# casys-kaist/CoVA

Hardware: AMD Instinct MI355X
Metric: compressed-domain frames/sec (BlobNet+bboxcc) at 1080p b=256 (higher is better)
Workload: dtype f16

## Files before the change

cova_amd/_lib.py:

```python
from __future__ import annotations

import ctypes as C
import os

import numpy as np

_HERE = os.path.dirname(os.path.abspath(__file__))
LIB_PATH = os.path.join(_HERE, "libcovahip.so")

OK = 0
MEM_HOST, MEM_DEVICE = 0, 1
AU_DELTA_UNIT, AU_DISCONT, AU_DROPPABLE = 1, 2, 4


class CovahipError(RuntimeError):
    def __init__(self, status: int, where: str, detail: str = ""):
        self.status = status
        try:
            text = lib().covahip_strerror(status).decode()
        except AttributeError:
            text = "error"
        msg = f"{where}: {text} (status {status})"
        if detail:
            msg += f" [{detail}]"
# ... 208 lines not shown
    "covahip_train_create": (C.c_int, [_P, C.POINTER(TrainCfg), _P, _SZ, C.POINTER(_P)]),
    "covahip_train_step": (C.c_int, [_P, _P, _P, C.c_int, C.c_float, C.POINTER(C.c_float), C.c_int]),
    "covahip_train_metrics": (C.c_int, [_P, C.POINTER(C.c_int64)]),
    "covahip_train_weights": (C.c_int, [_P, _P, _SZ, C.POINTER(_SZ)]),
    "covahip_train_grads": (C.c_int, [_P, _P, _SZ]),
    "covahip_train_create_set": (C.c_int, [_P, C.POINTER(TrainCfg), C.c_int, _P, _P, _P, C.POINTER(_P)]),
    "covahip_train_num_models": (C.c_int, [_P, C.POINTER(C.c_int)]),
    "covahip_train_step_set": (C.c_int, [_P, _P, _P, _P, _P, _P, C.c_int]),
    "covahip_train_metrics_m": (C.c_int, [_P, C.c_int, C.POINTER(C.c_int64)]),
    "covahip_train_weights_m": (C.c_int, [_P, C.c_int, _P, _SZ, C.POINTER(_SZ)]),
    "covahip_train_grads_m": (C.c_int, [_P, C.c_int, _P, _SZ]),
    "covahip_train_eval": (C.c_int, [_P, _P, _P, C.c_int, _P, _P, C.POINTER(TrainEvalResult), C.c_int]),
    "covahip_train_eval_set": (C.c_int, [_P, _P, _P, _P, _P, _P, C.POINTER(TrainEvalResult), C.c_int]),
    "covahip_train_state_size": (C.c_int, [_P, C.POINTER(_SZ)]),
    "covahip_train_save_state": (C.c_int, [_P, C.c_uint64, _P, _SZ, C.POINTER(_SZ)]),
    "covahip_train_load_state": (C.c_int, [_P, _P, _SZ, C.POINTER(C.c_uint64)]),
    "covahip_train_set_plan": (C.c_int, [_P, C.POINTER(TrainPlan)]),
    "covahip_train_get_plan": (C.c_int, [_P, C.POINTER(TrainPlan)]),
    "covahip_train_set_post": (C.c_int, [_P, C.c_int, C.POINTER(BlobNetPost)]),
    "covahip_train_get_post": (C.c_int, [_P, C.c_int, C.POINTER(C.c_float), _P, C.POINTER(C.c_int)]),
    "covahip_train_destroy": (None, [_P]),
    "covahip_train_data_create": (C.c_int, [_P, C.c_int, C.c_int, C.c_int64, C.POINTER(_P)]),
    "covahip_train_data_append": (C.c_int, [_P, _P, _P, C.c_int, C.c_int, C.POINTER(C.c_int64)]),
    "covahip_train_data_frames": (C.c_int, [_P, C.POINTER(C.c_int64)]),
    "covahip_train_data_gather": (C.c_int, [_P, _P, C.c_int, _P, _P, C.c_int]),
    "covahip_train_data_destroy": (None, [_P]),
    "covahip_train_step_data": (C.c_int, [_P, _P, _P, C.c_int, C.c_float, C.POINTER(C.c_float)]),
    "covahip_train_step_set_data": (C.c_int, [_P, _P, _P, _P, _P, _P]),
    "covahip_train_eval_data": (C.c_int, [_P, _P, _P, C.c_int, _P, _P, C.POINTER(TrainEvalResult), C.c_int]),
    "covahip_train_eval_set_data": (C.c_int, [_P, _P, _P, _P, _P, _P, C.POINTER(TrainEvalResult), C.c_int]),
    "covahip_post_sweep": (C.c_int, [_P, C.POINTER(SweepCfg), _P, _P, C.c_int, C.c_int, _P, _P, _P, C.POINTER(SweepResult)]),
    "covahip_post_heat_begin": (C.c_int, [_P, C.POINTER(HeatCfg)]),
    "covahip_post_heat_add": (C.c_int, [_P, _P, _P, C.c_int, C.c_int]),
    "covahip_post_heat_end": (C.c_int, [_P, _P, _P, _P, C.POINTER(C.c_int64)]),
    "covahip_monitor_begin": (C.c_int, [_P, C.POINTER(MonitorCfg)]),
    "covahip_monitor_add": (C.c_int, [_P, _P, _P, _P, _P, C.c_int, C.c_int]),
    "covahip_monitor_read": (C.c_int, [_P, C.c_int, _P, _P, _P, _P, _P, _P, C.POINTER(C.c_int64), C.POINTER(C.c_int64)]),
    "covahip_monitor_end": (C.c_int, [_P]),
    "covahip_mog_default_cfg": (None, [C.POINTER(MogCfg)]),
    "covahip_mog_create": (C.c_int, [_P, C.POINTER(MogCfg), C.POINTER(_P)]),
    "covahip_mog_create_grid": (C.c_int, [_P, C.POINTER(MogCfg), C.c_int, C.POINTER(_P)]),
    "covahip_mog_dims": (C.c_int, [_P, C.POINTER(C.c_int32), C.POINTER(C.c_int32), C.POINTER(C.c_int32), C.POINTER(C.c_int32)]),
    "covahip_mog_apply": (C.c_int, [_P, _P, C.c_int, _P, _P, C.c_int]),
    "covahip_mog_yuv_tight": (C.c_int, [_P, C.c_int, C.c_int, C.POINTER(MogYuv)]),
    "covahip_mog_apply_yuv": (C.c_int, [_P, C.POINTER(MogYuv), _P, C.c_int, _P, _P, C.c_int]),
    "covahip_mog_reset": (C.c_int, [_P, C.c_int]),
    "covahip_mog_destroy": (None, [_P]),
}

DEV_PROTOTYPES = {
    "covahip_blobnet_set_impl": (C.c_int, [_P, C.c_int]),
    "covahip_bboxcc_set_wave_cap": (C.c_int, [_P, C.c_int]),
    "covahip_blobnet_set_enc_plan": (C.c_int, [_P, C.c_int, C.c_int, C.c_int]),
    "covahip_dev_clock_mhz": (C.c_int, [_P, C.c_int, C.POINTER(C.c_float)]),
    "covahip_dev_graph_probe": (C.c_int, [_P, _P, C.c_int, _P, C.c_int, C.c_int, _P, _P, C.c_int, _P, C.c_int, C.POINTER(C.c_float),
                                          C.POINTER(C.c_float)]),
    "covahip_dev_bboxcc_overflow": (C.c_int, [_P, C.POINTER(C.c_int32)]),
    "covahip_dev_blobnet_tail_form": (C.c_int, [_P, C.POINTER(C.c_int)]),
    "covahip_dev_pipe_queue_plan": (C.c_int, [_P, C.POINTER(C.c_int), C.POINTER(C.c_int)]),
    "covahip_dev_blobnet_buffer": (C.c_int, [_P, C.c_int, C.c_int, C.POINTER(C.c_void_p), C.POINTER(C.c_size_t), C.POINTER(C.c_int32)]),
    "covahip_dev_mog_masks": (C.c_int, [_P, _P, _P, _SZ, C.POINTER(C.c_int)]),
    "covahip_dev_mog_state": (C.c_int, [_P, C.c_int, _P, _P, _P, _P, C.POINTER(C.c_int64)]),
    "covahip_dev_mog_set_stage_budget": (C.c_int, [_P, _SZ]),
    "covahip_dev_mog_post_masks": (C.c_int, [_P, _P, C.c_int, _P]),
    "covahip_dev_mog_set_post_form": (C.c_int, [_P, C.c_int, C.c_int]),
    "covahip_dev_mog_band_plan": (C.c_int, [C.c_int, C.c_int, C.POINTER(C.c_int), C.POINTER(C.c_int), C.POINTER(C.c_size_t)]),
    "covahip_dev_monitor_slice": (C.c_int, [_P, C.c_int]),
    "covahip_dev_heat_set_stage": (C.c_int, [_P, _SZ]),
    "covahip_dev_train_data_set_stage": (C.c_int, [_P, _SZ]),
}

_lib = None


def lib() -> C.CDLL:
    global _lib
    if _lib is None:
        san = os.environ.get("COVAHIP_HOST_SAN_LIB")
        if san:
            L = C.CDLL(san)
            for name, (res, args) in list(PROTOTYPES.items()) + list(DEV_PROTOTYPES.items()):
                fn = getattr(L, name, None)
                if fn is not None:
                    fn.restype = res
                    fn.argtypes = args
            _lib = L
            return _lib
        if not os.path.exists(LIB_PATH):
            raise ImportError(
                f"{LIB_PATH} not found: build it with `python -c 'import __graft_entry__ as g; g.build()'` "
                "or `make -C cova_amd/csrc` -- cova_amd has no CPU fallback")
        L = C.CDLL(LIB_PATH)
        for name, (res, args) in list(PROTOTYPES.items()) + list(DEV_PROTOTYPES.items()):
            fn = getattr(L, name)
            fn.restype = res
            fn.argtypes = args
        _lib = L
    return _lib


def check(status: int, where: str, ctx=None) -> None:
    if status != OK:
        detail = ""
        if ctx is not None and status == 3:
            detail = lib().covahip_last_hip_error(ctx).decode()
        raise CovahipError(status, where, detail)
# ... 1 lines not shown
```

cova_amd/csrc/blobnet.hip:

```cpp
#include <algorithm>
#include <cmath>
#include <cstdlib>
#include <cstring>
#include <vector>

#include "blobnet.h"
#include "covahip_dev.h"

static void free_model(covahip_ctx *ctx, covahip_blobnet *m) {
    if (!m) return;
    blobnet_release_mfma(ctx, m);
    if (m->d_post) hipFree(m->d_post);
    for (BnWorkspace &ws : m->ws) {
        for (int i = 0; i <= BN_LEVELS; i++)
            if (ws.act[i]) hipFree(ws.act[i]);
        for (int j = 0; j < BN_LEVELS; j++)
            if (ws.dact[j]) hipFree(ws.dact[j]);
        if (ws.pbuf) hipFree(ws.pbuf);
        if (ws.part) hipFree(ws.part);
        ws.index.release();
        ws.models.release();
        ws.areas.release();
    }
    delete m;
// ... 325 lines not shown
    m->post_thr[model] = post ? post->logit_thresh : 0.f;
    m->post_keep[model].clear();
    if (post && post->keep) {
        m->post_keep[model].resize(hw);
        for (size_t i = 0; i < hw; i++) m->post_keep[model][i] = post->keep[i] ? 1 : 0;
    }
    return commit_post(ctx, m);
}

int covahip_blobnet_set_area(covahip_ctx *ctx, int model, int area_thresh) {
    if (!ctx) return COVAHIP_ERR_INVALID_ARG;
    covahip_blobnet *m = ctx->blobnet;
    if (!m) return COVAHIP_ERR_NOT_LOADED;
    if (model < 0 || model >= m->n_models || area_thresh < 0) return COVAHIP_ERR_INVALID_ARG;
    COVAHIP_CHECK_HIP(ctx, hipSetDevice(ctx->device));
    if (int rc = covahip_sync_all(ctx)) return rc;
    m->post_area[model] = area_thresh;
    return commit_post(ctx, m);
}

int covahip_blobnet_get_area(covahip_ctx *ctx, int model, int *area_thresh) {
    if (!ctx || !area_thresh) return COVAHIP_ERR_INVALID_ARG;
    covahip_blobnet *m = ctx->blobnet;
    if (!m) return COVAHIP_ERR_NOT_LOADED;
    if (model < 0 || model >= m->n_models) return COVAHIP_ERR_INVALID_ARG;
    *area_thresh = m->post_area[model];
    return COVAHIP_OK;
}

int covahip_blobnet_get_post(covahip_ctx *ctx, int model, float *logit_thresh, uint8_t *keep_or_null, int *has_keep) {
    if (!ctx) return COVAHIP_ERR_INVALID_ARG;
    covahip_blobnet *m = ctx->blobnet;
    if (!m) return COVAHIP_ERR_NOT_LOADED;
    if (model < 0 || model >= m->n_models) return COVAHIP_ERR_INVALID_ARG;
    const std::vector<uint8_t> &keep = m->post_keep[model];
    if (logit_thresh) *logit_thresh = m->post_thr[model];
    if (has_keep) *has_keep = keep.empty() ? 0 : 1;
    if (keep_or_null) {
        const size_t hw = (size_t)m->H * m->W;
        if (keep.empty()) std::memset(keep_or_null, 1, hw);
        else std::memcpy(keep_or_null, keep.data(), hw);
    }
    return COVAHIP_OK;
}

int covahip_blobnet_macs_per_frame(covahip_ctx *ctx, int64_t *macs) {
    if (!ctx || !macs) return COVAHIP_ERR_INVALID_ARG;
    if (!ctx->blobnet) return COVAHIP_ERR_NOT_LOADED;
    *macs = ctx->blobnet->macs_per_frame;
    return COVAHIP_OK;
}

int covahip_blobnet_set_enc_plan(covahip_ctx *ctx, int level, int nbands, int nbuf) {
    if (!ctx || level < 1 || level > 3 || nbands < 0 || nbands > 64 || (nbands && nbuf != 1 && nbuf != 2)) return COVAHIP_ERR_INVALID_ARG;
    ctx->enc_plan[level].nbands = nbands;
    ctx->enc_plan[level].nbuf = nbands ? nbuf : 0;
    return COVAHIP_OK;
}

int covahip_blobnet_set_impl(covahip_ctx *ctx, int impl) {
    if (!ctx || !ctx->blobnet) return COVAHIP_ERR_NOT_LOADED;
    if (impl != 1 && (impl < 4 || impl > 10)) return COVAHIP_ERR_INVALID_ARG;
    ctx->blobnet->fuse_dec = impl != 4;
    ctx->blobnet->enc1_tile16 = impl != 5;
    ctx->blobnet->enc_rowtiles = impl != 6;
    ctx->blobnet->fuse_enc23 = impl == 7 ? 0 : impl == 8 ? 2 : 1;
    ctx->blobnet->tail_part = impl != 9;
    ctx->blobnet->tail_rows = impl != 10;
    return COVAHIP_OK;
}

static int filter_placed(covahip_ctx *ctx, covahip_blobnet *m, const uint8_t *d_src, int n_frames, const int32_t *stack_index,
                         int batch, int area_thresh, covahip_box *d_boxes, int32_t *d_counts, int max_boxes, float *d_logits,
                         uint8_t *d_mask, bool packed = false, const uint8_t *model_ids = nullptr) {
    if (!d_mask) {
        CtxLane &l = ctx->lane();
        int rc = covahip_ensure_buffer(ctx, &l.cc_scratch, &l.cc_scratch_bytes, (size_t)batch * m->H * m->W);
        if (rc) return rc;
        d_mask = (uint8_t *)l.cc_scratch;
    }
    BnInput in;
    if (n_frames > 0) {
        int rc = prepare_frames(ctx, m, m->ws[ctx->cur_lane], d_src, n_frames, stack_index, batch, in, model_ids);
        if (rc) return rc;
        in.packed = packed;
    } else {
        in.stack = d_src;
    }
    int rc = filter_dev(ctx, in, batch, d_logits, d_mask, true, area_thresh, d_boxes, d_counts, max_boxes, n_frames > 0 ? nullptr : model_ids);
    if (rc == COVAHIP_OK && batch > 0 && ctx->mon && ctx->mon->attached && !ctx->mon_suspended)
        rc = covahip_monitor_hook(ctx, d_mask, d_counts, d_boxes, max_boxes, model_ids, batch);
    return rc;
}

static int filter_any(covahip_ctx *ctx, const uint8_t *src, int n_frames, const int32_t *stack_index, int batch,
                      int area_thresh, covahip_box *boxes, int32_t *counts, int max_boxes, float *logits, uint8_t *mask,
                      int mem_kind, const uint8_t *model_ids = nullptr) {
    if (!ctx || batch < 0 || max_boxes < 0 || n_frames < 0) return COVAHIP_ERR_INVALID_ARG;
    covahip_blobnet *m = ctx->blobnet;
    if (!m) return COVAHIP_ERR_NOT_LOADED;
    if (batch == 0) return COVAHIP_OK;
    if (!src || !counts || (!boxes && max_boxes > 0) || batch > m->max_batch) return COVAHIP_ERR_INVALID_ARG;
    if (int rc = check_model_ids(m, model_ids, batch)) return rc;
    COVAHIP_CHECK_HIP(ctx, hipSetDevice(ctx->device));
    const bool by_frames = n_frames > 0;
    const size_t hw = (size_t)m->H * m->W;
    const size_t in_bytes = by_frames ? (size_t)n_frames * hw * 4 : (size_t)batch * BN_T * hw * 4;
// ... 223 lines not shown
```

cova_amd/csrc/blobnet_mfma.hip:

```cpp
#include <algorithm>
#include <cmath>
#include <cstdlib>
#include <cstring>
#include <mutex>
#include <type_traits>
#include <utility>
#include <vector>

#include "bboxcc_body.h"
#include "bboxcc_wave.h"
#include "blobnet.h"
#include "covahip_dev.h"

typedef _Float16 half8 __attribute__((ext_vector_type(8)));
typedef _Float16 half4 __attribute__((ext_vector_type(4)));
typedef float f32x16 __attribute__((ext_vector_type(16)));
typedef float f32x4 __attribute__((ext_vector_type(4)));
typedef _Float16 half2v __attribute__((ext_vector_type(2)));

namespace {

constexpr float BN_EPS = 1e-3f;
constexpr int WG = 256;

// ... 239 lines not shown
    }
}

#ifdef PHASE_TIMING
__device__ unsigned long long g_phase[80];
#define PHASE_MARK(i)                                                     \
    do {                                                                  \
        const unsigned long long now_ = __builtin_amdgcn_s_memrealtime(); \
        ph_[i] += now_ - last_;                                           \
        last_ = now_;                                                     \
    } while (0)
#else
#define PHASE_MARK(i) do { } while (0)
#endif
#if defined(PHASE_TIMING) || defined(WGSPAN_ONLY)
__device__ unsigned long long g_wgspan[6][1024][4];
#define WGSPAN_BEGIN() const unsigned long long wg_t0_ = __builtin_amdgcn_s_memrealtime(), wg_c0_ = __builtin_amdgcn_s_memtime()
#define WGSPAN_END(kid)                                                                          \
    do {                                                                                         \
        if (threadIdx.x == 0 && blockIdx.x < 1024) {                                             \
            g_wgspan[kid][blockIdx.x][0] = wg_t0_;                                               \
            g_wgspan[kid][blockIdx.x][1] = __builtin_amdgcn_s_memrealtime();                     \
            g_wgspan[kid][blockIdx.x][2] = __builtin_amdgcn_s_getreg(4 | (0 << 6) | (31 << 11)); \
            g_wgspan[kid][blockIdx.x][3] = __builtin_amdgcn_s_memtime() - wg_c0_;                \
        }                                                                                        \
    } while (0)
#else
#define WGSPAN_BEGIN() do { } while (0)
#define WGSPAN_END(kid) do { } while (0)
#endif
#ifdef WGSPAN_ONLY
__device__ unsigned long long g_itemspan[3][1024][4][4];
#define ITEM_MARK(j) do { if (it_n_ < 4) it_t_[it_n_][j] = __builtin_amdgcn_s_memrealtime(); } while (0)
#else
#define ITEM_MARK(j) do { } while (0)
#endif
constexpr int WG0 = 512;
struct Enc0pArgs {
    const uint8_t *in;
    __half *out;
    const half8 *wfrag;
    const float *epi;
    int F, H, W, Hp, Wp, Ho, Wo, oy, ox;
    int nbands, TC;
    uint32_t mWp, mNb, mW4;
    int scr_off;
    const uint8_t *model_ids;
    uint32_t mstride;
};
template <bool ALLPOS, bool PACKED, bool MS = false>
__global__ __launch_bounds__(WG0, 4) void enc0p_mfma(Enc0pArgs p) {
    extern __shared__ __attribute__((aligned(16))) uint8_t smem[];
    WGSPAN_BEGIN();
    const int tid = threadIdx.x, lane = tid & 63, wave = tid >> 6;
    const int TC = p.TC;
    half8 be0 = p.wfrag[lane], be1 = p.wfrag[64 + lane];
    half8 bo0 = p.wfrag[128 + lane], bo1 = p.wfrag[192 + lane];
    const int co = lane & 15;
    float e0 = p.epi[co], e1 = p.epi[16 + co], e2 = p.epi[32 + co];
    [[maybe_unused]] uint32_t moff_cur = 0;
    const int m = lane & 15, g = lane >> 4;
    const uint32_t lc0 = (uint32_t)((((m & 1) + (g >> 1)) * TC + 2 * (m >> 1) + 2 * (g & 1)) * 8);
    const uint32_t lc1 = (uint32_t)((((m & 1) + 2) * TC + 2 * (m >> 1) + 2 * (g & 1)) * 8);
    const int n_items = p.F * p.nbands;
    for (int item = blockIdx.x; item < n_items; item += gridDim.x) {
        const int f = fdiv(item, p.mNb), band = item - f * p.nbands;
        if constexpr (MS) {
            const uint32_t mo = model_off<MS>(p.model_ids, p.mstride, f);
            if (mo != moff_cur) {
                moff_cur = mo;
                const half8 *wf = at_model(p.wfrag, mo);
                const float *ep = at_model(p.epi, mo);
                be0 = wf[lane]; be1 = wf[64 + lane]; bo0 = wf[128 + lane]; bo1 = wf[192 + lane];
                e0 = ep[co]; e1 = ep[16 + co]; e2 = ep[32 + co];
            }
        }
        const int y0 = 2 * ((band * p.Hp) / p.nbands);
        const int rows = 2 * (((band + 1) * p.Hp) / p.nbands) - y0;
        const int n2 = rows + 2;
        lds_barrier();
        {
            const int W4 = p.W >> 2;
            const int per_t = n2 * W4;
            const uint8_t *fb = p.in + (size_t)f * p.H * p.W * (PACKED ? 2 : 4);
            uint4 v[2];
            int dsto[2];
#pragma unroll
            for (int k = 0; k < 2; k++) {
                const int i = tid + k * WG0;
                dsto[k] = -1;
                v[k] = make_uint4(0, 0, 0, 0);
                if (i < per_t) {
                    const int r = fdiv(i, p.mW4), c4 = i - r * W4;
                    const int y = y0 - 1 + r;
                    dsto[k] = r * TC * 8 + 16 + c4 * 32;
                    if (y >= 0 && y < p.H) {
                        if constexpr (PACKED) {
                            const uint2 w = *reinterpret_cast<const uint2 *>(fb + ((size_t)y * p.W + c4 * 4) * 2);
                            v[k].x = w.x; v[k].y = w.y;
                        } else {
                            v[k] = *reinterpret_cast<const uint4 *>(fb + ((size_t)y * p.W + c4 * 4) * 4);
                        }
                    }
                }
            }
            const half2v clip = {(_Float16)1030.f, (_Float16)1030.f}, off = {(_Float16)1024.f, (_Float16)1024.f};
#pragma unroll
            for (int k = 0; k < 2; k++) {
                if (dsto[k] >= 0) {
                    uint32_t o[8];
                    if constexpr (PACKED) {
                        const uint32_t pw[2] = {v[k].x, v[k].y};
#pragma unroll
                        for (int q = 0; q < 4; q++) {
                            const uint32_t r = (pw[q >> 1] >> (16 * (q & 1))) & 0xFFFFu;
                            const uint32_t c01 = 0x64006400u | (r & 7u) | (((r >> 3) & 7u) << 16);
                            const uint32_t c23 = 0x64006400u | ((r >> 6) & 7u);
                            o[2 * q] = __builtin_bit_cast(uint32_t, __builtin_bit_cast(half2v, c01) - off);
                            o[2 * q + 1] = __builtin_bit_cast(uint32_t, __builtin_bit_cast(half2v, c23) - off);
                        }
                    } else {
                        const uint32_t px[4] = {v[k].x, v[k].y, v[k].z, v[k].w};
#pragma unroll
                        for (int q = 0; q < 4; q++) {
                            const uint32_t c01 = __builtin_amdgcn_perm(0x64646464u, px[q], 0x05010500u);
                            const uint32_t c23 = __builtin_amdgcn_perm(0x64646464u, px[q], 0x05030502u);
                            const half2v h01 = __builtin_elementwise_min(__builtin_bit_cast(half2v, c01), clip) - off;
                            const half2v h23 = __builtin_elementwise_min(__builtin_bit_cast(half2v, c23), clip) - off;
                            o[2 * q] = __builtin_bit_cast(uint32_t, h01);
                            o[2 * q + 1] = __builtin_bit_cast(uint32_t, h23);
                        }
                    }
                    uint8_t *d = smem + dsto[k];
                    *reinterpret_cast<uint4 *>(d) = make_uint4(o[0], o[1], o[2], o[3]);
                    *reinterpret_cast<uint4 *>(d + 16) = make_uint4(o[4], o[5], o[6], o[7]);
                }
            }
            for (int i = tid; i < n2 * 2; i += WG0)
                *reinterpret_cast<uint4 *>(smem + (i >> 1) * TC * 8 + ((i & 1) ? (p.W + 2) * 8 : 0)) = make_uint4(0, 0, 0, 0);
        }
        lds_barrier();
        const int nhalf = (p.Wp + 31) >> 5;
        const int ngroups = (rows / 2) * nhalf;
        uint8_t *const scr = smem + p.scr_off + wave * 1024;
        __half *const ob = p.out + (size_t)f * p.Ho * p.Wo * 16;
        int g_wy = 0, g_h = wave;
        for (int grp = wave; grp < ngroups; grp += WG0 / 64, g_h += WG0 / 64) {
            while (g_h >= nhalf) { g_h -= nhalf; g_wy++; }
            const uint32_t gbase = (uint32_t)(((2 * g_wy) * TC + 64 * g_h) * 8);
            const uint8_t *const a0 = smem + (gbase + lc0), *const a1 = smem + (gbase + lc1);
#pragma unroll
            for (int k = 0; k < 4; k++) {
                const half8 ae0 = *reinterpret_cast<const half8 *>(__builtin_assume_aligned(a0 + k * 128, 16));
                const half8 ae1 = *reinterpret_cast<const half8 *>(__builtin_assume_aligned(a1 + k * 128, 16));
                const half8 ao0 = *reinterpret_cast<const half8 *>(__builtin_assume_aligned(a0 + k * 128 + 16, 16));
                const half8 ao1 = *reinterpret_cast<const half8 *>(__builtin_assume_aligned(a1 + k * 128 + 16, 16));
                f32x4 ce = {0.f, 0.f, 0.f, 0.f}, co_ = {0.f, 0.f, 0.f, 0.f};
                ce = __builtin_amdgcn_mfma_f32_16x16x32_f16(ae0, be0, ce, 0, 0, 0);
                co_ = __builtin_amdgcn_mfma_f32_16x16x32_f16(ao0, bo0, co_, 0, 0, 0);
                ce = __builtin_amdgcn_mfma_f32_16x16x32_f16(ae1, be1, ce, 0, 0, 0);
                co_ = __builtin_amdgcn_mfma_f32_16x16x32_f16(ao1, bo1, co_, 0, 0, 0);
                _Float16 *sw = reinterpret_cast<_Float16 *>(scr + (k * 8 + 2 * g) * 32) + co;
                float v0 = pool4<ALLPOS>(ce[0], ce[1], co_[0], co_[1], e0, e1, e2);
                float v1 = pool4<ALLPOS>(ce[2], ce[3], co_[2], co_[3], e0, e1, e2);
                asm volatile("" : "+v"(v0), "+v"(v1));
                sw[0] = (_Float16)v0;
                sw[16] = (_Float16)v1;
            }
            __builtin_amdgcn_fence(__ATOMIC_RELEASE, "wavefront");
            __builtin_amdgcn_wave_barrier();
            __builtin_amdgcn_fence(__ATOMIC_ACQUIRE, "wavefront");
            const int owx = 32 * g_h + (lane >> 1);
            if (owx < p.Wp) {
                const int gy = y0 / 2 + g_wy + p.oy, gx = owx + p.ox;
                *reinterpret_cast<uint4 *>(ob + (gy * p.Wo + gx) * 16 + 8 * (lane & 1)) =
                    *reinterpret_cast<const uint4 *>(scr + lane * 16);
            }
            __builtin_amdgcn_fence(__ATOMIC_RELEASE, "wavefront");
            __builtin_amdgcn_wave_barrier();
        }
    }
    WGSPAN_END(5);
}

template <int CIN, int COUT, int TPAR, int OCC, int NWV, bool WIDE, bool ALLPOS, bool PRE = false, int TSZ = 0, bool MS = false>
__global__ __launch_bounds__(NWV * 64, OCC) void enc_mfma(EncArgs p) {
    constexpr int WGS = NWV * 64;
    constexpr int NT = COUT / 32, MG = NWV / NT, KC = CIN / 16, KSTEPS = 9 * KC;
    constexpr int CPP = CIN / 8, PS = CIN * 2;
    constexpr int AD = CIN == 32 ? 8 : 0;
    extern __shared__ __attribute__((aligned(16))) uint8_t smem[];
    const int tid = threadIdx.x, lane = tid & 63, wave = tid >> 6;
    const int ntile = wave % NT, mgroup = wave / NT;
    const int TR = p.TR, TC = p.TC;
    const int tsz = TSZ > 0 ? TSZ : TR * TC * PS;
    static_assert(TSZ == 0 || (TSZ % 16 == 0 && (TPAR - 1) * TSZ < 65536 && !PRE), "T-slice offsets must fit a DS instruction's offset field");

    WGSPAN_BEGIN();
#ifdef PHASE_TIMING
    unsigned long long ph_[9] = {0, 0, 0, 0, 0, 0, 0, 0, 0}, last_ = __builtin_amdgcn_s_memrealtime();
    asm volatile("s_waitcnt lgkmcnt(0)" ::: "memory");
#endif
    auto mlp_own = [&](uint8_t *base, int band_, const TmixW &tmp) {
        const int n2_ = 2 * (((band_ + 1) * p.Hp) / p.nbands) - 2 * ((band_ * p.Hp) / p.nbands) + 2;
        const int nchunk = n2_ * TC * CPP;
        for (int sidx = tid; sidx < nchunk; sidx += WGS) {
            half8 v[BN_T], o[BN_T];
#pragma unroll
            for (int t = 0; t < BN_T; t++) v[t] = *reinterpret_cast<const half8 *>(base + t * tsz + sidx * 16);
#pragma unroll
            for (int j0 = 0; j0 < 8; j0 += 4) {
                half4 pb[4];
                f32x4 r[4];
#pragma unroll
                for (int j = 0; j < 4; j++) pb[j] = half4{v[0][j0 + j], v[1][j0 + j], v[2][j0 + j], v[3][j0 + j]};
                tmix4f<4>(tmp, pb, r);
#pragma unroll
                for (int j = 0; j < 4; j++)
#pragma unroll
                    for (int t = 0; t < BN_T; t++) o[t][j0 + j] = (_Float16)r[j][t];
            }
#pragma unroll
            for (int t = 0; t < BN_T; t++) *reinterpret_cast<half8 *>(base + t * tsz + sidx * 16) = o[t];
        }
    };
    auto stage = [&](int sb, int sband, uint8_t *dst, int ll) {
        const int sy0 = 2 * ((sband * p.Hp) / p.nbands);
        const int sn2 = 2 * (((sband + 1) * p.Hp) / p.nbands) - sy0 + 2;
        int fidx[BN_T] = {0, 1, 2, 3};
        if constexpr (PRE) {
            typedef int i32x4 __attribute__((ext_vector_type(4)));
            typedef const __attribute__((address_space(4))) i32x4 *const_i32x4_ptr;
            if (p.pidx) {
// ... 1988 lines not shown

void blobnet_release_mfma(covahip_ctx *, covahip_blobnet *m) {
    if (m->d_prepared) hipFree(m->d_prepared);
    m->d_prepared = nullptr;
    delete m->prep;
    m->prep = nullptr;
}

namespace {

struct Fwd {
    covahip_ctx *ctx;
    const covahip_blobnet *m;
    const Prepared *pr;
    BnWorkspace &ws;
    const BnInput &inp;
    int batch;
    const uint8_t *prep;
    uint32_t mstride;
    bool ms;
    bool dry;
    bool by_frames;
    int num_cu;
    const uint8_t *d_frames;
    int n_frames;
    const int32_t *d_index;
    float *d_logits;
    uint8_t *d_mask;
    const BnCcTail *cc;
    bool part_written = false;
    bool post = false;
    DecPost pp{};
};

template <bool POST>
PostArg<POST> post_arg(const Fwd &f) {
    if constexpr (POST) return f.pp;
    else return DecNoPost{};
}

template <typename K, typename... A>
int launch(const Fwd &f, const char *name, K kernel, int grid, int block, size_t lds, const A &...args) {
    if (int rc = covahip_open_lds(f.ctx, kernel, lds, LDS_LIMIT)) return rc;
    ProfScope ps(f.ctx, name);
    if (!f.dry) hipLaunchKernelGGL(kernel, dim3(grid), dim3(block), lds, f.ctx->stream, args...);
    return COVAHIP_OK;
}
int launched(const Fwd &f, int rc) {
    if (rc) return rc;
    COVAHIP_CHECK_HIP(f.ctx, hipGetLastError());
    return COVAHIP_OK;
}

int run_enc0p(const Fwd &f) {
    const covahip_blobnet *m = f.m;
    const Prepared *pr = f.pr;
    const int H = m->lv[0].H, W = m->lv[0].W, Hp = H / 2, Wp = W / 2;
    const int TC = ((W + 4 - 16 + 31) / 32) * 32 + 16;
    if (W % 4) return COVAHIP_ERR_UNSUPPORTED;
    int nbands = 0;
    for (int nb = 1; nb <= Hp; nb++) {
        const int rb = (Hp + nb - 1) / nb, n2 = 2 * rb + 2;
        if (n2 * (W / 4) > 2 * WG0 || (size_t)n2 * TC * 8 > 30 * 1024) continue;
        if ((long long)f.n_frames * nb < 2LL * f.num_cu && nb < Hp) continue;
        nbands = nb;
        break;
    }
    if (!nbands) return COVAHIP_ERR_UNSUPPORTED;
    const int rbmax = (Hp + nbands - 1) / nbands;
    const size_t tile_bytes = (((size_t)(2 * rbmax + 2) * TC * 8) + 15) & ~(size_t)15;
    Enc0pArgs a;
    a.in = f.d_frames; a.out = f.ws.pbuf;
    a.wfrag = (const half8 *)(f.prep + pr->enc[0].wfrag); a.epi = (const float *)(f.prep + pr->enc[0].epi);
    a.F = f.n_frames; a.H = H; a.W = W; a.Hp = Hp; a.Wp = Wp; a.Ho = m->lv[1].H; a.Wo = m->lv[1].W;
    a.oy = H & 1; a.ox = W & 1; a.nbands = nbands; a.TC = TC;
    a.mWp = magic(Wp); a.mNb = magic(nbands); a.mW4 = magic(W / 4); a.scr_off = (int)tile_bytes;
    a.model_ids = f.inp.frame_models; a.mstride = f.mstride;
    const size_t lds = tile_bytes + (size_t)(WG0 / 64) * 1024;
    const int grid = std::min(f.n_frames * nbands, 3 * f.num_cu);
    return launched(f, with_bools([&](auto AP, auto PACKED, auto MS) {
        return launch(f, "enc0p_mfma", enc0p_mfma<AP.value, PACKED.value, MS.value>, grid, WG0, lds, a);
    }, pr->allpos[0], f.inp.packed, f.ms));
}

bool run_enc1_tile16(Fwd &f, int &rc) {
    const covahip_blobnet *m = f.m;
    const Prepared *pr = f.pr;
    if (!bn_level1_on_enc1(f.ctx, m)) return false;
    const int H = m->lv[1].H, W = m->lv[1].W, Hp = H / 2, Wp = W / 2;
    const int nbands = plan_bands(Hp, f.batch, 2LL * f.num_cu, [](int rb) { return 2 * rb + 2 <= E1_TR; });
    if (!nbands) return false;
    Enc1Args a;
    a.in = f.ws.pbuf; a.out = f.ws.act[2];
    a.wfrag = (const half8 *)(f.prep + pr->enc1w); a.epi = (const float *)(f.prep + pr->enc[1].epi);
    a.B = f.batch; a.H = H; a.W = W; a.Hp = Hp; a.Wp = Wp; a.Ho = m->lv[2].H; a.Wo = m->lv[2].W;
    a.oy = H & 1; a.ox = W & 1; a.nbands = nbands;
    a.mWp = magic(Wp); a.mRC = magic(2 * (W + 2));
    a.scr_off = BN_T * E1_TSZ;
    const int grid = std::min(f.batch * nbands, 2 * f.num_cu);
    a.plan = make_plan(grid, f.num_cu, 2, f.batch, nbands, Hp);
    a.pidx = f.d_index; a.skip = f.ws.act[1]; a.tm_pre = (const float *)(f.prep + pr->enc[0].epi) + 48;
    f.part_written = m->tail_part && f.ws.part && m->dec_ci[3] == 32 && m->dec_co[3] == 16 && m->enc_c[1] == 16;
    a.part = f.part_written ? f.ws.part : nullptr;
    a.wtail = (const half8 *)(f.prep + pr->tail_w);
    a.mXe = magic(2 * Wp);
    a.use_ktab = 0;
    if (f.by_frames && f.inp.h_index && f.batch <= BN_KTAB_STACKS) {
        a.use_ktab = 1;
        for (int k = 0; k < f.batch * BN_T; k++) a.ktab[k] = (uint16_t)f.inp.h_index[k];
    } else if (f.by_frames && !f.d_index && !f.dry) {
        rc = COVAHIP_ERR_INVALID_ARG;
        return true;
    }
    const size_t lds = (size_t)BN_T * E1_TSZ + 8 * 1024 + E1_CONST;
    a.model_ids = f.inp.model_ids; a.mstride = f.mstride;
    rc = launched(f, with_bools([&](auto AP, auto MS) {
        return launch(f, "enc1_mfma", enc1_mfma<AP.value, MS.value>, grid, 512, lds, a);
    }, pr->allpos[1], f.ms));
    return true;
}

bool run_enc23(const Fwd &f, int &rc) {
    const covahip_blobnet *m = f.m;
    const Prepared *pr = f.pr;
    if (!(m->fuse_enc23 && m->enc_rowtiles && !f.ctx->enc_plan[2].nbands && !f.ctx->enc_plan[3].nbands && m->enc_c[2] == 32 &&
          m->enc_c[3] == 64 && m->enc_c[4] == 128))
        return false;
    const int H = m->lv[2].H, W = m->lv[2].W, Hp = H / 2, Wp = W / 2;
    const int H3 = m->lv[3].H, W3 = m->lv[3].W, Hp3 = H3 / 2, Wp3 = W3 / 2;
    const size_t lds = (size_t)BN_T * E3_TSZ + (size_t)BN_T * E23_TSZ2 + 4096;
    const bool pays = 4 * f.batch >= 3 * f.num_cu && 20 * Wp >= 17 * 8 * ((Wp + 7) / 8) && 20 * Wp3 >= 17 * 8 * ((Wp3 + 7) / 8);
    if (!((pays || m->fuse_enc23 == 2 || f.ms) && (W + 2) * 64 <= E23_RP2 && Wp <= 16 && Hp >= 1 && Hp3 >= 1 && Wp3 >= 1 &&
// ... 244 lines not shown
}

int blobnet_forward_mfma(covahip_ctx *ctx, covahip_blobnet *m, BnWorkspace &ws, const BnInput &inp, int batch, float *d_logits,
                         uint8_t *d_mask, const BnCcTail *cc, bool *cc_done) {
    if (cc_done) *cc_done = false;
    const Prepared *pr = m->prep;
    const bool dry = inp.dry;
    const bool by_frames = inp.frames != nullptr || (dry && inp.n_frames > 0);
    const bool ms = inp.model_ids != nullptr || (dry && inp.mixed);
    Fwd f{ctx, m, pr, ws, inp, batch,
          (const uint8_t *)m->d_prepared + (ms ? 0 : (size_t)inp.model * pr->total), (uint32_t)pr->total,
          ms, dry, by_frames, ctx->props.multiProcessorCount,
          by_frames ? inp.frames : inp.stack, by_frames ? inp.n_frames : batch * BN_T, by_frames ? inp.index : nullptr,
          d_logits, d_mask, cc};
    if ((size_t)f.n_frames > ws.pbuf_frames && !dry) return COVAHIP_ERR_INVALID_ARG;
    f.post = m->post_on;
    if (f.post) {
        if (!m->d_post) return COVAHIP_ERR_INVALID_ARG;
        const uint8_t *const dp = (const uint8_t *)m->d_post;
        const size_t k = ms ? 0 : (size_t)inp.model;
        f.pp.thr = m->post_thr[k];
        f.pp.thr_tab = (const float *)dp;
        f.pp.area = m->post_area[k] >= 1 ? m->post_area[k] : (cc ? cc->area_thresh : 0);
        f.pp.area_tab = (const int32_t *)(dp + m->post_area_off);
        f.pp.keep = dp + m->post_keep_off + k * m->post_keep_stride;
        f.pp.planes = (const uint32_t *)(dp + m->post_planes_off + k * m->post_planes_stride);
        f.pp.keep_stride = (uint32_t)m->post_keep_stride;
        f.pp.planes_stride = (uint32_t)m->post_planes_stride;
    }

    int rc = run_enc0p(f);
    if (rc) return rc;
    if (!run_enc1_tile16(f, rc)) rc = run_enc_level(f, 1);
    if (rc) return rc;
    if (!run_enc23(f, rc)) {
        rc = run_enc_level(f, 2);
        if (!rc) rc = run_enc_level(f, 3);
    }
    if (rc) return rc;
    if (!run_dec012(f, rc))
        for (int j = 0; j < BN_LEVELS - 1 && !rc; j++) rc = run_dec_block(f, j);
    if (rc) return rc;
    DecPlan last;
    rc = plan_dec_block(f, BN_LEVELS - 1, last);
    if (rc) return rc;
    if (!(cc && m->fuse_tail && run_tail_fused(f, last))) {
        if (!dry) ctx->tail_form = COVAHIP_DEV_TAIL_ALONE;
        return launch_dec_block(f, BN_LEVELS - 1, last);
    }
    if (cc_done) *cc_done = true;
    return launched(f, COVAHIP_OK);
}

#if defined(PHASE_TIMING) || defined(WGSPAN_ONLY)
extern "C" int covahip_dev_wgspan_read(unsigned long long *out, int kid) {
    return hipMemcpyFromSymbol(out, HIP_SYMBOL(g_wgspan), sizeof(unsigned long long) * 1024 * 4, sizeof(unsigned long long) * 1024 * 4 * kid) != hipSuccess;
}
#endif
#ifdef WGSPAN_ONLY
extern "C" int covahip_dev_itemspan_read(unsigned long long *out, int kid) {
    return hipMemcpyFromSymbol(out, HIP_SYMBOL(g_itemspan), sizeof(unsigned long long) * 1024 * 16, sizeof(unsigned long long) * 1024 * 16 * kid) != hipSuccess;
}
#endif
#ifdef PHASE_TIMING
extern "C" int covahip_dev_ccphase_read(unsigned long long *out8, int reset) {
    if (hipMemcpyFromSymbol(out8, HIP_SYMBOL(g_ccph), sizeof(g_ccph)) != hipSuccess) return 1;
    if (reset) {
        unsigned long long z[8] = {0};
        if (hipMemcpyToSymbol(HIP_SYMBOL(g_ccph), z, sizeof(z)) != hipSuccess) return 1;
    }
    return 0;
}
extern "C" int covahip_dev_phase_read(unsigned long long *out64, int reset) {
    if (hipMemcpyFromSymbol(out64, HIP_SYMBOL(g_phase), sizeof(g_phase)) != hipSuccess) return 1;
    if (reset) {
        unsigned long long z[80] = {0};
        if (hipMemcpyToSymbol(HIP_SYMBOL(g_phase), z, sizeof(z)) != hipSuccess) return 1;
    }
    return 0;
}
#endif
```

include/covahip_dev.h:

```cpp
#ifndef COVAHIP_DEV_H
#define COVAHIP_DEV_H

#include "covahip.h"

#ifdef __cplusplus
extern "C" {
#endif

int covahip_blobnet_set_impl(covahip_ctx *ctx, int impl);

int covahip_bboxcc_set_wave_cap(covahip_ctx *ctx, int cap);
int covahip_dev_bboxcc_overflow(covahip_ctx *ctx, int32_t *out4);

int covahip_blobnet_set_enc_plan(covahip_ctx *ctx, int level, int nbands, int nbuf);

int covahip_dev_blobnet_buffer(covahip_ctx *ctx, int which, int index, void **dptr, size_t *bytes, int32_t dims[5]);

int covahip_dev_clock_mhz(covahip_ctx *ctx, int busy_us, float *mhz);

int covahip_dev_graph_probe(covahip_ctx *ctx, const uint8_t *d_frames, int n_frames, const int32_t *stack_index, int batch,
                            int area_thresh, covahip_box *d_boxes, int32_t *d_counts, int max_boxes, uint8_t *d_mask, int iters,
                            float *ms_direct, float *ms_graph);

#define COVAHIP_DEV_TAIL_ALONE 1
#define COVAHIP_DEV_TAIL_ROWS 2
#define COVAHIP_DEV_TAIL_BANDS 4
int covahip_dev_blobnet_tail_form(covahip_ctx *ctx, int *form);

struct covahip_pipe;
int covahip_dev_pipe_queue_plan(struct covahip_pipe *pipe, int *lanes_on_upload_queue, int *lanes_on_result_queue);

struct covahip_mog;
int covahip_dev_mog_masks(struct covahip_mog *m, uint8_t *raw, uint8_t *filled, size_t cap, int *n_frames);
int covahip_dev_mog_state(struct covahip_mog *m, int stream, float *W, float *V, float *M, uint8_t *nmodes, int64_t *n);
int covahip_dev_mog_set_stage_budget(struct covahip_mog *m, size_t bytes);
int covahip_dev_mog_post_masks(struct covahip_mog *m, const uint8_t *raw, int n_frames, uint8_t *labels);
int covahip_dev_mog_set_post_form(struct covahip_mog *m, int banded, int band_rows);
int covahip_dev_mog_band_plan(int work_w, int work_h, int *rows, int *bands, size_t *lds_bytes);

int covahip_dev_monitor_slice(covahip_ctx *ctx, int samples);

int covahip_dev_heat_set_stage(covahip_ctx *ctx, size_t bytes);
struct covahip_train_data;
int covahip_dev_train_data_set_stage(struct covahip_train_data *data, size_t bytes);

#ifdef __cplusplus
}
#endif
#endif
```

Baseline: 2.437 million.

## Prefetch next band's input into registers during enc0p MFMA compute and replan grid

The enc0p kernel now issues the global loads for the next band item into registers before computing the current one, so memory latency overlaps with MFMA work instead of stalling at the start of each item. Grid sizing moves into a planner that targets 4 workgroups per CU and picks a band count that divides evenly into rounds, replacing the fixed 3×CU cap. The planner also adds override knobs and a debug entry point. This adds register pressure for the prefetched data and an extra barrier per iteration.

```diff
diff --git a/cova_amd/_lib.py b/cova_amd/_lib.py
--- a/cova_amd/_lib.py
+++ b/cova_amd/_lib.py
@@ -284,6 +284,7 @@
     "covahip_blobnet_set_impl": (C.c_int, [_P, C.c_int]),
     "covahip_bboxcc_set_wave_cap": (C.c_int, [_P, C.c_int]),
     "covahip_blobnet_set_enc_plan": (C.c_int, [_P, C.c_int, C.c_int, C.c_int]),
+    "covahip_dev_enc0p_plan": (C.c_int, [C.c_int, C.c_int, C.c_int, C.c_int, C.c_int, C.c_int, C.POINTER(C.c_int32)]),
     "covahip_dev_clock_mhz": (C.c_int, [_P, C.c_int, C.POINTER(C.c_float)]),
     "covahip_dev_graph_probe": (C.c_int, [_P, _P, C.c_int, _P, C.c_int, C.c_int, _P, _P, C.c_int, _P, C.c_int, C.POINTER(C.c_float),
                                           C.POINTER(C.c_float)]),
diff --git a/cova_amd/csrc/blobnet.hip b/cova_amd/csrc/blobnet.hip
--- a/cova_amd/csrc/blobnet.hip
+++ b/cova_amd/csrc/blobnet.hip
@@ -401,7 +401,8 @@
 }
 
 int covahip_blobnet_set_enc_plan(covahip_ctx *ctx, int level, int nbands, int nbuf) {
-    if (!ctx || level < 1 || level > 3 || nbands < 0 || nbands > 64 || (nbands && nbuf != 1 && nbuf != 2)) return COVAHIP_ERR_INVALID_ARG;
+    if (!ctx || level < 0 || level > 3 || nbands < 0 || nbands > 64) return COVAHIP_ERR_INVALID_ARG;
+    if (nbands && (level ? nbuf != 1 && nbuf != 2 : nbuf < 1 || (nbuf > 8 && nbuf < 12) || nbuf > 14)) return COVAHIP_ERR_INVALID_ARG;
     ctx->enc_plan[level].nbands = nbands;
     ctx->enc_plan[level].nbuf = nbands ? nbuf : 0;
     return COVAHIP_OK;
diff --git a/cova_amd/csrc/blobnet_mfma.hip b/cova_amd/csrc/blobnet_mfma.hip
--- a/cova_amd/csrc/blobnet_mfma.hip
+++ b/cova_amd/csrc/blobnet_mfma.hip
@@ -315,7 +315,8 @@
 __global__ __launch_bounds__(WG0, 4) void enc0p_mfma(Enc0pArgs p) {
     extern __shared__ __attribute__((aligned(16))) uint8_t smem[];
     WGSPAN_BEGIN();
-    const int tid = threadIdx.x, lane = tid & 63, wave = tid >> 6;
+    const int tid = threadIdx.x, lane = tid & 63;
+    const int wave = __builtin_amdgcn_readfirstlane(tid >> 6);
     const int TC = p.TC;
     half8 be0 = p.wfrag[lane], be1 = p.wfrag[64 + lane];
     half8 bo0 = p.wfrag[128 + lane], bo1 = p.wfrag[192 + lane];
@@ -326,8 +327,48 @@
     const uint32_t lc0 = (uint32_t)((((m & 1) + (g >> 1)) * TC + 2 * (m >> 1) + 2 * (g & 1)) * 8);
     const uint32_t lc1 = (uint32_t)((((m & 1) + 2) * TC + 2 * (m >> 1) + 2 * (g & 1)) * 8);
     const int n_items = p.F * p.nbands;
-    for (int item = blockIdx.x; item < n_items; item += gridDim.x) {
+    const int W4 = p.W >> 2;
+    struct Band { int f, y0, rows; };
+    auto band_of = [&](int item) {
         const int f = fdiv(item, p.mNb), band = item - f * p.nbands;
+        const int y0 = 2 * ((band * p.Hp) / p.nbands);
+        return Band{f, y0, 2 * (((band + 1) * p.Hp) / p.nbands) - y0};
+    };
+    uint4 v[2];
+    uint32_t dsto = 0;
+    constexpr uint32_t NONE = 0xFFFFu;
+    auto request = [&](const Band &bd) {
+        const int per_t = (bd.rows + 2) * W4;
+        const uint8_t *fb = p.in + (size_t)bd.f * p.H * p.W * (PACKED ? 2 : 4);
+        int t = tid;
+        asm volatile("" : "+v"(t));
+        dsto = NONE | (NONE << 16);
+#pragma unroll
+        for (int k = 0; k < 2; k++) {
+            const int i = t + k * WG0;
+            v[k] = make_uint4(0, 0, 0, 0);
+            if (i < per_t) {
+                const int r = fdiv(i, p.mW4), c4 = i - r * W4;
+                const int y = bd.y0 - 1 + r;
+                const uint32_t d = (uint32_t)(r * TC * 8 + 16 + c4 * 32);
+                dsto = k ? (dsto & 0xFFFFu) | (d << 16) : (dsto & 0xFFFF0000u) | d;
+                if (y >= 0 && y < p.H) {
+                    if constexpr (PACKED) {
+                        const uint2 w = *reinterpret_cast<const uint2 *>(fb + ((size_t)y * p.W + c4 * 4) * 2);
+                        v[k].x = w.x; v[k].y = w.y;
+                    } else {
+                        v[k] = *reinterpret_cast<const uint4 *>(fb + ((size_t)y * p.W + c4 * 4) * 4);
+                    }
+                }
+            }
+        }
+    };
+    int item = blockIdx.x;
+    if (item >= n_items) return;
+    Band cur = band_of(item);
+    request(cur);
+    for (;;) {
+        const int f = cur.f, y0 = cur.y0, rows = cur.rows;
         if constexpr (MS) {
             const uint32_t mo = model_off<MS>(p.model_ids, p.mstride, f);
             if (mo != moff_cur) {
@@ -338,39 +379,14 @@
                 e0 = ep[co]; e1 = ep[16 + co]; e2 = ep[32 + co];
             }
         }
-        const int y0 = 2 * ((band * p.Hp) / p.nbands);
-        const int rows = 2 * (((band + 1) * p.Hp) / p.nbands) - y0;
         const int n2 = rows + 2;
-        lds_barrier();
+        wait_vmem();
         {
-            const int W4 = p.W >> 2;
-            const int per_t = n2 * W4;
-            const uint8_t *fb = p.in + (size_t)f * p.H * p.W * (PACKED ? 2 : 4);
-            uint4 v[2];
-            int dsto[2];
+            const half2v clip = {(_Float16)1030.f, (_Float16)1030.f}, off = {(_Float16)1024.f, (_Float16)1024.f};
 #pragma unroll
             for (int k = 0; k < 2; k++) {
-                const int i = tid + k * WG0;
-                dsto[k] = -1;
-                v[k] = make_uint4(0, 0, 0, 0);
-                if (i < per_t) {
-                    const int r = fdiv(i, p.mW4), c4 = i - r * W4;
-                    const int y = y0 - 1 + r;
-                    dsto[k] = r * TC * 8 + 16 + c4 * 32;
-                    if (y >= 0 && y < p.H) {
-                        if constexpr (PACKED) {
-                            const uint2 w = *reinterpret_cast<const uint2 *>(fb + ((size_t)y * p.W + c4 * 4) * 2);
-                            v[k].x = w.x; v[k].y = w.y;
-                        } else {
-                            v[k] = *reinterpret_cast<const uint4 *>(fb + ((size_t)y * p.W + c4 * 4) * 4);
-                        }
-                    }
-                }
-            }
-            const half2v clip = {(_Float16)1030.f, (_Float16)1030.f}, off = {(_Float16)1024.f, (_Float16)1024.f};
-#pragma unroll
-            for (int k = 0; k < 2; k++) {
-                if (dsto[k] >= 0) {
+                const uint32_t dk = k ? dsto >> 16 : dsto & 0xFFFFu;
+                if (dk != NONE) {
                     uint32_t o[8];
                     if constexpr (PACKED) {
                         const uint32_t pw[2] = {v[k].x, v[k].y};
@@ -394,15 +410,23 @@
                             o[2 * q + 1] = __builtin_bit_cast(uint32_t, h23);
                         }
                     }
-                    uint8_t *d = smem + dsto[k];
+                    uint8_t *d = smem + dk;
                     *reinterpret_cast<uint4 *>(d) = make_uint4(o[0], o[1], o[2], o[3]);
                     *reinterpret_cast<uint4 *>(d + 16) = make_uint4(o[4], o[5], o[6], o[7]);
                 }
             }
-            for (int i = tid; i < n2 * 2; i += WG0)
+            int t = tid;
+            asm volatile("" : "+v"(t));
+            for (int i = t; i < n2 * 2; i += WG0)
                 *reinterpret_cast<uint4 *>(smem + (i >> 1) * TC * 8 + ((i & 1) ? (p.W + 2) * 8 : 0)) = make_uint4(0, 0, 0, 0);
         }
         lds_barrier();
+        item += gridDim.x;
+        const bool more = item < n_items;
+        if (more) {
+            cur = band_of(item);
+            request(cur);
+        }
         const int nhalf = (p.Wp + 31) >> 5;
         const int ngroups = (rows / 2) * nhalf;
         uint8_t *const scr = smem + p.scr_off + wave * 1024;
@@ -442,6 +466,8 @@
             __builtin_amdgcn_fence(__ATOMIC_RELEASE, "wavefront");
             __builtin_amdgcn_wave_barrier();
         }
+        if (!more) break;
+        lds_barrier();
     }
     WGSPAN_END(5);
 }
@@ -2536,23 +2562,58 @@
     return COVAHIP_OK;
 }
 
+constexpr int ENC0P_WGS_PER_CU = 4;
+struct Enc0pPlan {
+    int nbands = 0;
+    int grid = 0, TC = 0;
+    size_t tile_bytes = 0, lds_bytes = 0;
+};
+Enc0pPlan plan_enc0p(int H, int W, int n_frames, int num_cu, int ov_nb, int ov_mode) {
+    Enc0pPlan pl;
+    const int Hp = H / 2;
+    if (W % 4 || Hp < 1 || n_frames < 1 || num_cu < 1) return pl;
+    const int TC = ((W + 4 - 16 + 31) / 32) * 32 + 16;
+    auto fits = [&](int nb) {
+        const int rb = (Hp + nb - 1) / nb, n2 = 2 * rb + 2;
+        return n2 * (W / 4) <= 2 * WG0 && (size_t)n2 * TC * 8 <= 30 * 1024;
+    };
+    int nb_fill = 0;
+    for (int nb = 1; nb <= Hp && !nb_fill; nb++)
+        if (fits(nb) && ((long long)n_frames * nb >= 2LL * num_cu || nb == Hp)) nb_fill = nb;
+    if (!nb_fill) return pl;
+    int nbands = nb_fill;
+    long long grid = (long long)n_frames * nbands;
+    if (ov_nb) {
+        nbands = std::min(ov_nb, Hp);
+        if (!fits(nbands)) return pl;
+        const long long items = (long long)n_frames * nbands;
+        grid = ov_mode >= 12 ? std::min(items, (long long)(ov_mode - 10) * num_cu) : (items + std::max(ov_mode, 1) - 1) / std::max(ov_mode, 1);
+    } else if (grid > (long long)ENC0P_WGS_PER_CU * num_cu) {
+        const long long slots = (long long)ENC0P_WGS_PER_CU * num_cu;
+        auto rounds = [&](int nb) { return ((long long)n_frames * nb + slots - 1) / slots; };
+        for (int nb = nb_fill; nb <= std::min(nb_fill + 2, Hp); nb++)
+            if (fits(nb) && ((long long)n_frames * nb) % rounds(nb) == 0) {
+                nbands = nb;
+                break;
+            }
+        grid = ((long long)n_frames * nbands + rounds(nbands) - 1) / rounds(nbands);
+    }
+    if (grid > 0x7fffffffLL) return pl;
+    pl.nbands = nbands; pl.grid = (int)grid; pl.TC = TC;
+    const int rbmax = (Hp + nbands - 1) / nbands;
+    pl.tile_bytes = (((size_t)(2 * rbmax + 2) * TC * 8) + 15) & ~(size_t)15;
+    pl.lds_bytes = pl.tile_bytes + (size_t)(WG0 / 64) * 1024;
+    return pl;
+}
+
 int run_enc0p(const Fwd &f) {
     const covahip_blobnet *m = f.m;
     const Prepared *pr = f.pr;
     const int H = m->lv[0].H, W = m->lv[0].W, Hp = H / 2, Wp = W / 2;
-    const int TC = ((W + 4 - 16 + 31) / 32) * 32 + 16;
-    if (W % 4) return COVAHIP_ERR_UNSUPPORTED;
-    int nbands = 0;
-    for (int nb = 1; nb <= Hp; nb++) {
-        const int rb = (Hp + nb - 1) / nb, n2 = 2 * rb + 2;
-        if (n2 * (W / 4) > 2 * WG0 || (size_t)n2 * TC * 8 > 30 * 1024) continue;
-        if ((long long)f.n_frames * nb < 2LL * f.num_cu && nb < Hp) continue;
-        nbands = nb;
-        break;
-    }
-    if (!nbands) return COVAHIP_ERR_UNSUPPORTED;
-    const int rbmax = (Hp + nbands - 1) / nbands;
-    const size_t tile_bytes = (((size_t)(2 * rbmax + 2) * TC * 8) + 15) & ~(size_t)15;
+    const Enc0pPlan pl = plan_enc0p(H, W, f.n_frames, f.num_cu, f.ctx->enc_plan[0].nbands, f.ctx->enc_plan[0].nbuf);
+    if (!pl.nbands) return COVAHIP_ERR_UNSUPPORTED;
+    const int nbands = pl.nbands, grid = pl.grid, TC = pl.TC;
+    const size_t tile_bytes = pl.tile_bytes;
     Enc0pArgs a;
     a.in = f.d_frames; a.out = f.ws.pbuf;
     a.wfrag = (const half8 *)(f.prep + pr->enc[0].wfrag); a.epi = (const float *)(f.prep + pr->enc[0].epi);
@@ -2560,8 +2621,7 @@
     a.oy = H & 1; a.ox = W & 1; a.nbands = nbands; a.TC = TC;
     a.mWp = magic(Wp); a.mNb = magic(nbands); a.mW4 = magic(W / 4); a.scr_off = (int)tile_bytes;
     a.model_ids = f.inp.frame_models; a.mstride = f.mstride;
-    const size_t lds = tile_bytes + (size_t)(WG0 / 64) * 1024;
-    const int grid = std::min(f.n_frames * nbands, 3 * f.num_cu);
+    const size_t lds = pl.lds_bytes;
     return launched(f, with_bools([&](auto AP, auto PACKED, auto MS) {
         return launch(f, "enc0p_mfma", enc0p_mfma<AP.value, PACKED.value, MS.value>, grid, WG0, lds, a);
     }, pr->allpos[0], f.inp.packed, f.ms));
@@ -2912,6 +2972,14 @@
     return launched(f, COVAHIP_OK);
 }
 
+int covahip_dev_enc0p_plan(int h_mb, int w_mb, int n_frames, int num_cu, int nbands, int mode, int32_t out4[4]) {
+    if (!out4 || nbands < 0 || nbands > 64 || mode < 0 || mode > 14) return COVAHIP_ERR_INVALID_ARG;
+    const Enc0pPlan pl = plan_enc0p(h_mb, w_mb, n_frames, num_cu, nbands, mode);
+    if (!pl.nbands) return COVAHIP_ERR_UNSUPPORTED;
+    out4[0] = pl.nbands; out4[1] = pl.grid; out4[2] = (int32_t)pl.tile_bytes; out4[3] = (int32_t)pl.lds_bytes;
+    return COVAHIP_OK;
+}
+
 #if defined(PHASE_TIMING) || defined(WGSPAN_ONLY)
 extern "C" int covahip_dev_wgspan_read(unsigned long long *out, int kid) {
     return hipMemcpyFromSymbol(out, HIP_SYMBOL(g_wgspan), sizeof(unsigned long long) * 1024 * 4, sizeof(unsigned long long) * 1024 * 4 * kid) != hipSuccess;
diff --git a/include/covahip_dev.h b/include/covahip_dev.h
--- a/include/covahip_dev.h
+++ b/include/covahip_dev.h
@@ -13,6 +13,8 @@
 int covahip_dev_bboxcc_overflow(covahip_ctx *ctx, int32_t *out4);
 
 int covahip_blobnet_set_enc_plan(covahip_ctx *ctx, int level, int nbands, int nbuf);
+
+int covahip_dev_enc0p_plan(int h_mb, int w_mb, int n_frames, int num_cu, int nbands, int mode, int32_t out4[4]);
 
 int covahip_dev_blobnet_buffer(covahip_ctx *ctx, int which, int index, void **dptr, size_t *bytes, int32_t dims[5]);
 
```

After: 2.444 million (median of 3 runs). Within noise of the previous version (+0.3%).
